# Arlo0o/StereoScene

Measured on AMD Instinct MI355X. Metric: voxels/sec fwd+bwd, 256x256x32 grid D=192, higher is better.
Workload: dtype f32; 1 GPU; kitti_d192: stereo pair features 2x[B,640,48,160] -> 256x256x32 occupancy, D=192, fwd+bwd incl. 4 losses; batch_per_gpu=1, global_batch=1, parallelism=dp1, train_mode=True

## Files before the change

### include/ssbev.h

```cpp
#ifndef SSBEV_H
#define SSBEV_H

#include <stddef.h>
#include <stdint.h>

#ifdef __cplusplus
extern "C" {
#endif

#define SSBEV_OK 0
#define SSBEV_EINVAL (-1)
#define SSBEV_EWORKSPACE (-2)
#define SSBEV_ELAUNCH (-3)

typedef void* ssbev_stream_t;

int ssbev_version(void);
const char* ssbev_build_arch(void);
void ssbev_env_refresh(void);

typedef struct {
  int B;
  int P;
  int C;
// ... 36 lines not shown
                         const int32_t* vox, float* grad_depth, float* grad_feat,
                         const ssbev_pool_dims* d, const ssbev_lift_dims* l, ssbev_stream_t stream);

typedef struct { int B, C, G, D, H, W; float down; int align_corners; } ssbev_gwc_dims;
int ssbev_gwc_warp_fwd(const float* left, const float* right, const float* calib, float* vol,
                       const ssbev_gwc_dims* d, ssbev_stream_t stream);
int ssbev_gwc_warp_bwd(const float* grad_vol, const float* left, const float* right,
                       const float* calib, float* grad_left, float* grad_right,
                       const ssbev_gwc_dims* d, ssbev_stream_t stream);
size_t ssbev_gwc_warp_bwd_workspace(const ssbev_gwc_dims* d);
int ssbev_gwc_warp_bwd_fused(const float* grad_vol, const float* left, const float* right,
                             const float* calib, float* grad_left, float* grad_right,
                             const ssbev_gwc_dims* d, void* workspace, size_t ws_bytes, ssbev_stream_t stream);

typedef struct {
  int B, Cin, Cout;
  int Di, Hi, Wi;
  int Do, Ho, Wo;
  int kd, kh, kw;
  int sd, sh, sw;
  int pd, ph, pw;
  int dd, dh, dw;
  int transposed;
  int relu;
  int accumulate;
  int tile_hint;
  int precision;
} ssbev_conv_dims;

size_t ssbev_conv_packed_weight_elems(const ssbev_conv_dims* d);
int ssbev_conv_kernel_class(const ssbev_conv_dims* d, int mode);
int ssbev_conv_chunk_groups(const ssbev_conv_dims* d, int mode);

size_t ssbev_conv_thin_workspace(const ssbev_conv_dims* d, int mode);
size_t ssbev_conv_thin_packed_elems(const ssbev_conv_dims* d, int mode);
int ssbev_conv_thin_pack(const float* w_src, float* w_packed, const ssbev_conv_dims* d, int mode, ssbev_stream_t stream);
int ssbev_conv_thin_run(const float* x, const float* w_packed, const float* bias, float* y, const ssbev_conv_dims* d,
                        int mode, void* workspace, size_t ws_bytes, ssbev_stream_t stream);
int ssbev_conv_pack_weight(const float* w_src, float* w_packed, const ssbev_conv_dims* d, int mode,
                           ssbev_stream_t stream);
int ssbev_conv_fwd(const float* x, const float* w_packed, const float* bias, float* y,
                   const ssbev_conv_dims* d, ssbev_stream_t stream);
int ssbev_conv_fwd_bf16(const uint16_t* x, const float* w_packed, const float* bias, void* y,
                        const ssbev_conv_dims* d, ssbev_stream_t stream);
int ssbev_conv_bwd_data_bf16(const uint16_t* gy, const float* w_packed_t, void* gx,
                             const ssbev_conv_dims* d, ssbev_stream_t stream);
int ssbev_conv_bwd_weight_bf16(const uint16_t* x, const uint16_t* gy, float* gw, const ssbev_conv_dims* d,
                               void* ws, size_t ws_bytes, ssbev_stream_t stream);
int ssbev_conv_bwd_data(const float* gy, const float* w_packed_t, float* gx,
                        const ssbev_conv_dims* d, ssbev_stream_t stream);
size_t ssbev_conv_bwd_weight_workspace(const ssbev_conv_dims* d);
int ssbev_conv_bwd_weight(const float* x, const float* gy, float* gw, const ssbev_conv_dims* d,
                          void* ws, size_t ws_bytes, ssbev_stream_t stream);

typedef struct { int M, N, K, batch; int out_fp32; } ssbev_gemm16_dims;
size_t ssbev_gemm16_packed_elems(const ssbev_gemm16_dims* d);
int ssbev_gemm16_pack(const float* B, uint16_t* packed, const ssbev_gemm16_dims* d, ssbev_stream_t stream);
int ssbev_gemm16_nn(const uint16_t* A, const uint16_t* packed, void* C, const ssbev_gemm16_dims* d, ssbev_stream_t stream);
size_t ssbev_gemm16_tn_workspace(const ssbev_gemm16_dims* d);
int ssbev_gemm16_tn(const uint16_t* A, const uint16_t* B, float* C, const ssbev_gemm16_dims* d, float* workspace,
                    size_t workspace_elems, ssbev_stream_t stream);

typedef struct { int B, C, G; int64_t S; float eps; int relu; int stats_given; int pre_act; int64_t ld_y, ld_gy; int io_dtype; } ssbev_norm_dims;
size_t ssbev_groupnorm_workspace(const ssbev_norm_dims* d);
int ssbev_groupnorm_fwd(const float* x, const float* gamma, const float* beta, const float* residual,
                        float* y, float* mean, float* rstd, const ssbev_norm_dims* d, void* ws,
                        size_t ws_bytes, ssbev_stream_t stream);
int ssbev_groupnorm_bwd(const float* gy, const float* x, const float* y, const float* gamma,
                        const float* mean, const float* rstd, float* gx, float* gresidual,
                        float* ggamma, float* gbeta, const ssbev_norm_dims* d, void* ws,
                        size_t ws_bytes, ssbev_stream_t stream);
size_t ssbev_groupnorm_mask_words(const ssbev_norm_dims* d);
int ssbev_groupnorm_fwd_mask(const float* x, const float* gamma, const float* beta, const float* residual, float* y,
                             float* mean, float* rstd, uint64_t* relu_mask, const ssbev_norm_dims* d, void* ws,
                             size_t ws_bytes, ssbev_stream_t stream);
int ssbev_groupnorm_bwd_mask(const float* gy, const float* x, const uint64_t* relu_mask, const float* gamma,
                             const float* mean, const float* rstd, float* gx, float* gresidual, float* ggamma, float* gbeta,
                             const ssbev_norm_dims* d, void* ws, size_t ws_bytes, ssbev_stream_t stream);

typedef struct { float* running_mean; float* running_var; float momentum; int64_t n; } ssbev_norm_ext;
int ssbev_groupnorm_fwd_ext(const float* x, const float* gamma, const float* beta, const float* residual, float* y,
                            float* mean, float* rstd, uint64_t* relu_mask, const ssbev_norm_dims* d,
                            const ssbev_norm_ext* ext, void* ws, size_t ws_bytes, ssbev_stream_t stream);
int ssbev_groupnorm_bwd_ext(const float* gy, const float* x, const float* y, const uint64_t* relu_mask, const float* gamma,
                            const float* mean, const float* rstd, float* gx, float* gresidual, float* ggamma, float* gbeta,
                            const ssbev_norm_dims* d, const ssbev_norm_ext* ext, void* ws, size_t ws_bytes,
                            ssbev_stream_t stream);

typedef struct { int B, C, Ga, Gb; int64_t S; float eps_a, eps_b; int relu; int a_batch, b_batch; int io_dtype;  } ssbev_norm2_dims;
size_t ssbev_groupnorm2_workspace(const ssbev_norm2_dims* d);
int ssbev_groupnorm2_fwd(const float* xa, const float* gamma_a, const float* beta_a, float* mean_a, float* rstd_a,
                         const float* xb, const float* gamma_b, const float* beta_b, float* mean_b, float* rstd_b, float* y,
                         uint64_t* relu_mask, const ssbev_norm2_dims* d, void* ws, size_t ws_bytes, ssbev_stream_t stream);
int ssbev_groupnorm2_bwd(const float* gy, const uint64_t* relu_mask, const float* xa, const float* gamma_a, const float* mean_a,
                         const float* rstd_a, const float* xb, const float* gamma_b, const float* mean_b, const float* rstd_b,
                         float* gxa, float* gxb, float* ggamma_a, float* gbeta_a, float* ggamma_b, float* gbeta_b,
                         const ssbev_norm2_dims* d, void* ws, size_t ws_bytes, ssbev_stream_t stream);

typedef struct { float* running_mean_a; float* running_var_a; float momentum_a;
                 float* running_mean_b; float* running_var_b; float momentum_b; } ssbev_norm2_ext;
int ssbev_groupnorm2_fwd_ext(const float* xa, const float* gamma_a, const float* beta_a, float* mean_a, float* rstd_a,
                             const float* xb, const float* gamma_b, const float* beta_b, float* mean_b, float* rstd_b, float* y,
                             uint64_t* relu_mask, const ssbev_norm2_dims* d, const ssbev_norm2_ext* ext, void* ws, size_t ws_bytes,
                             ssbev_stream_t stream);
int ssbev_groupnorm2_bwd_ext(const float* gy, const uint64_t* relu_mask, const float* xa, const float* gamma_a, const float* mean_a,
                             const float* rstd_a, const float* xb, const float* gamma_b, const float* mean_b, const float* rstd_b,
// ... 214 lines not shown
```

### stereoscene_amd/capi.py

```python
import ctypes as C
import os

import torch

_HERE = os.path.dirname(os.path.abspath(__file__))
LIB_PATH = os.path.join(_HERE, "_lib", "libssbev_hip.so")

OK, EINVAL, EWORKSPACE, ELAUNCH = 0, -1, -2, -3
_ERR = {EINVAL: "SSBEV_EINVAL (bad dims / null pointer / unsupported configuration)",
        EWORKSPACE: "SSBEV_EWORKSPACE (workspace too small)",
        ELAUNCH: "SSBEV_ELAUNCH (HIP launch failure)"}


class SsbevError(RuntimeError):
    pass


class PoolDims(C.Structure):
    _fields_ = [("B", C.c_int), ("P", C.c_int), ("C", C.c_int), ("nx", C.c_int), ("ny", C.c_int), ("nz", C.c_int),
                ("origin", C.c_float * 3), ("dx", C.c_float * 3)]


class LiftDims(C.Structure):
    _fields_ = [("N", C.c_int), ("D", C.c_int), ("HW", C.c_int)]
# ... 78 lines not shown
    _fields_ = [("kernel", C.c_int), ("bm", C.c_int), ("bn", C.c_int), ("bk", C.c_int), ("nchunk", C.c_int), ("per_chunk", C.c_int),
                ("grid", C.c_int64), ("workspace", C.c_size_t)]


class JitterParams(C.Structure):
    _fields_ = [("flags", C.c_int), ("mode", C.c_int), ("delta", C.c_float), ("alpha", C.c_float), ("saturation", C.c_float),
                ("hue", C.c_float), ("perm", C.c_int * 3)]


JITTER_BRIGHTNESS, JITTER_CONTRAST, JITTER_SATURATION, JITTER_HUE, JITTER_SWAP = 1, 2, 4, 8, 16


class AdamWCfg(C.Structure):
    _fields_ = [("lr", C.c_float), ("beta1", C.c_float), ("beta2", C.c_float), ("eps", C.c_float),
                ("weight_decay", C.c_float), ("max_grad_norm", C.c_float), ("step", C.c_int)]


_P = C.c_void_p
SIGNATURES = {
    "ssbev_version": (C.c_int, []),
    "ssbev_build_arch": (C.c_char_p, []),
    "ssbev_env_refresh": (None, []),
    "ssbev_voxel_index": (C.c_int, [_P, _P, _P, C.POINTER(PoolDims), _P]),
    "ssbev_coords_to_vox": (C.c_int, [_P, C.c_int, _P, C.POINTER(PoolDims), _P]),
    "ssbev_pool_prepare_workspace": (C.c_size_t, [C.c_int, C.POINTER(PoolDims)]),
    "ssbev_pool_prepare": (C.c_int, [_P, C.c_int, _P, _P, C.POINTER(PoolDims), _P, C.c_size_t, _P]),
    "ssbev_pool_long_list_elems": (C.c_size_t, [C.c_int]),
    "ssbev_pool_prepare2": (C.c_int, [_P, C.c_int, _P, _P, _P, C.POINTER(PoolDims), _P, C.c_size_t, _P]),
    "ssbev_bev_pool_fwd": (C.c_int, [_P, _P, _P, _P, C.POINTER(PoolDims), _P]),
    "ssbev_bev_pool_bwd": (C.c_int, [_P, _P, C.c_int, _P, C.POINTER(PoolDims), _P]),
    "ssbev_lift_splat_fwd": (C.c_int, [_P, _P, _P, _P, _P, C.POINTER(PoolDims), C.POINTER(LiftDims), _P]),
    "ssbev_lift_splat_fwd2": (C.c_int, [_P, _P, _P, _P, _P, _P, C.POINTER(PoolDims), C.POINTER(LiftDims), _P]),
    "ssbev_lift_splat_bwd": (C.c_int, [_P, _P, _P, _P, _P, _P, C.POINTER(PoolDims), C.POINTER(LiftDims), _P]),
    "ssbev_gwc_warp_fwd": (C.c_int, [_P, _P, _P, _P, C.POINTER(GwcDims), _P]),
    "ssbev_gwc_warp_bwd": (C.c_int, [_P, _P, _P, _P, _P, _P, C.POINTER(GwcDims), _P]),
    "ssbev_gwc_warp_bwd_workspace": (C.c_size_t, [C.POINTER(GwcDims)]),
    "ssbev_gwc_warp_bwd_fused": (C.c_int, [_P, _P, _P, _P, _P, _P, C.POINTER(GwcDims), _P, C.c_size_t, _P]),
    "ssbev_conv_packed_weight_elems": (C.c_size_t, [C.POINTER(ConvDims)]),
    "ssbev_conv_kernel_class": (C.c_int, [C.POINTER(ConvDims), C.c_int]),
    "ssbev_conv_chunk_groups": (C.c_int, [C.POINTER(ConvDims), C.c_int]),
    "ssbev_frustum_geometry": (C.c_int, [_P] * 9 + [C.POINTER(GeomDims), _P]),
    "ssbev_conv_pack_weight": (C.c_int, [_P, _P, C.POINTER(ConvDims), C.c_int, _P]),
    "ssbev_conv_thin_workspace": (C.c_size_t, [C.POINTER(ConvDims), C.c_int]),
    "ssbev_conv_thin_packed_elems": (C.c_size_t, [C.POINTER(ConvDims), C.c_int]),
    "ssbev_conv_thin_pack": (C.c_int, [_P, _P, C.POINTER(ConvDims), C.c_int, _P]),
    "ssbev_conv_thin_run": (C.c_int, [_P, _P, _P, _P, C.POINTER(ConvDims), C.c_int, _P, C.c_size_t, _P]),
    "ssbev_conv_fwd": (C.c_int, [_P, _P, _P, _P, C.POINTER(ConvDims), _P]),
    "ssbev_conv_bwd_data": (C.c_int, [_P, _P, _P, C.POINTER(ConvDims), _P]),
    "ssbev_conv_fwd_bf16": (C.c_int, [_P, _P, _P, _P, C.POINTER(ConvDims), _P]),
    "ssbev_conv_bwd_data_bf16": (C.c_int, [_P, _P, _P, C.POINTER(ConvDims), _P]),
    "ssbev_conv_bwd_weight_bf16": (C.c_int, [_P, _P, _P, C.POINTER(ConvDims), _P, C.c_size_t, _P]),
    "ssbev_conv_bwd_weight_workspace": (C.c_size_t, [C.POINTER(ConvDims)]),
    "ssbev_conv_bwd_weight": (C.c_int, [_P, _P, _P, C.POINTER(ConvDims), _P, C.c_size_t, _P]),
    "ssbev_gemm16_packed_elems": (C.c_size_t, [C.POINTER(Gemm16Dims)]),
    "ssbev_gemm16_pack": (C.c_int, [_P, _P, C.POINTER(Gemm16Dims), _P]),
    "ssbev_gemm16_nn": (C.c_int, [_P, _P, _P, C.POINTER(Gemm16Dims), _P]),
    "ssbev_gemm16_tn_workspace": (C.c_size_t, [C.POINTER(Gemm16Dims)]),
    "ssbev_gemm16_tn": (C.c_int, [_P, _P, _P, C.POINTER(Gemm16Dims), _P, C.c_size_t, _P]),
    "ssbev_groupnorm_workspace": (C.c_size_t, [C.POINTER(NormDims)]),
    "ssbev_groupnorm_fwd": (C.c_int, [_P] * 7 + [C.POINTER(NormDims), _P, C.c_size_t, _P]),
    "ssbev_groupnorm_bwd": (C.c_int, [_P] * 10 + [C.POINTER(NormDims), _P, C.c_size_t, _P]),
    "ssbev_groupnorm_mask_words": (C.c_size_t, [C.POINTER(NormDims)]),
    "ssbev_groupnorm_fwd_mask": (C.c_int, [_P] * 8 + [C.POINTER(NormDims), _P, C.c_size_t, _P]),
    "ssbev_groupnorm_bwd_mask": (C.c_int, [_P] * 10 + [C.POINTER(NormDims), _P, C.c_size_t, _P]),
    "ssbev_groupnorm_fwd_ext": (C.c_int, [_P] * 8 + [C.POINTER(NormDims), C.POINTER(NormExt), _P, C.c_size_t, _P]),
    "ssbev_groupnorm_bwd_ext": (C.c_int, [_P] * 11 + [C.POINTER(NormDims), C.POINTER(NormExt), _P, C.c_size_t, _P]),
    "ssbev_groupnorm2_fwd_ext": (C.c_int, [_P] * 12 + [C.POINTER(Norm2Dims), C.POINTER(Norm2Ext), _P, C.c_size_t, _P]),
    "ssbev_groupnorm2_bwd_ext": (C.c_int, [_P] * 16 + [C.POINTER(Norm2Dims), C.POINTER(Norm2Ext), _P, C.c_size_t, _P]),
    "ssbev_groupnorm2_workspace": (C.c_size_t, [C.POINTER(Norm2Dims)]),
    "ssbev_groupnorm2_fwd": (C.c_int, [_P] * 12 + [C.POINTER(Norm2Dims), _P, C.c_size_t, _P]),
    "ssbev_groupnorm2_bwd": (C.c_int, [_P] * 16 + [C.POINTER(Norm2Dims), _P, C.c_size_t, _P]),
    "ssbev_groupnorm_plan_query": (C.c_int, [C.POINTER(NormDims), C.POINTER(Norm2Dims), C.c_int, C.POINTER(GroupnormPlan)]),
    "ssbev_trilinear2x_fwd": (C.c_int, [_P, _P, C.POINTER(UpsampleDims), _P]),
    "ssbev_trilinear2x_bwd": (C.c_int, [_P, _P, C.POINTER(UpsampleDims), _P]),
    "ssbev_dcn_im2col": (C.c_int, [_P, _P, _P, C.POINTER(DcnDims), _P]),
    "ssbev_dcn_col2im_workspace": (C.c_size_t, [C.POINTER(DcnDims)]),
    "ssbev_dcn_col2im": (C.c_int, [_P, _P, _P, _P, _P, C.POINTER(DcnDims), _P, C.c_size_t, _P]),
    "ssbev_bn_update_running": (C.c_int, [_P, _P, _P, _P, C.c_int, C.c_float, C.c_float, C.c_int64, _P]),
    "ssbev_resize_pil_u8": (C.c_int, [_P, C.c_int, C.c_int, C.c_int, _P, _P, C.c_int, _P, _P, C.c_int, _P, _P, C.c_int, C.c_int, _P]),
    "ssbev_crop_normalize_u8": (C.c_int, [_P, C.c_int, C.c_int, _P, C.c_int, C.c_int, C.c_int, C.c_int, C.c_int, _P, _P, C.c_int, _P]),
    "ssbev_crop_rotate_normalize_u8": (C.c_int, [_P, C.c_int, C.c_int, _P, C.c_int, C.c_int, C.c_int, C.c_int, C.c_int, _P, _P, _P,
                                                C.c_int, _P]),
    "ssbev_crop_rotate_jitter_normalize_u8": (C.c_int, [_P, C.c_int, C.c_int, _P, C.c_int, C.c_int, C.c_int, C.c_int, C.c_int, _P,
                                                       C.POINTER(JitterParams), _P, _P, C.c_int, _P]),
    "ssbev_depth_bce_workspace": (C.c_size_t, [C.c_int, C.c_int, C.c_int]),
    "ssbev_depth_bce_fwd": (C.c_int, [_P, _P, _P] + [C.c_int] * 5 + [C.c_float] * 3 + [_P, C.c_size_t, _P]),
    "ssbev_depth_bce_bwd": (C.c_int, [_P, _P, _P, _P] + [C.c_int] * 5 + [C.c_float] * 3 + [_P, _P]),
    "ssbev_lidar_depth_workspace": (C.c_size_t, [C.c_int, C.c_int]),
    "ssbev_lidar_depth_map": (C.c_int, [_P, C.c_int, _P, _P, _P, _P, _P, _P, C.c_int, C.c_int, _P, C.c_size_t, _P]),
    "ssbev_dwconv2d_fwd": (C.c_int, [_P, _P, _P, C.POINTER(DwDims), _P]),
    "ssbev_dwconv2d_bwd_data": (C.c_int, [_P, _P, _P, C.POINTER(DwDims), _P]),
    "ssbev_dwconv2d_bwd_weight_workspace": (C.c_size_t, [C.POINTER(DwDims)]),
    "ssbev_dwconv2d_bwd_weight": (C.c_int, [_P, _P, _P, C.POINTER(DwDims), _P, C.c_size_t, _P]),
    "ssbev_swish_fwd": (C.c_int, [_P, _P, C.c_int64, _P]),
    "ssbev_swish_bwd": (C.c_int, [_P, _P, _P, C.c_int64, _P]),
    "ssbev_chan_sum_workspace": (C.c_size_t, [C.c_int, C.c_int64, C.c_int]),
    "ssbev_chan_sum": (C.c_int, [_P, _P, _P, C.c_int, C.c_int64, C.c_int, C.c_float, _P, C.c_size_t, _P]),
    "ssbev_chan_scale": (C.c_int, [_P, _P, _P, C.c_int, C.c_int64, C.c_int, C.c_float, _P]),
    "ssbev_wino_input_transform": (C.c_int, [_P, _P, C.POINTER(WinoDims), _P]),
    "ssbev_wino_output_transform": (C.c_int, [_P, _P, C.POINTER(WinoDims), _P]),
    "ssbev_wino_output_adjoint": (C.c_int, [_P, _P, C.POINTER(WinoDims), _P]),
    "ssbev_wino_weight_transform": (C.c_int, [_P, _P, C.c_int, C.c_int, C.c_int, C.c_int, _P]),
    "ssbev_wino_weight_grad": (C.c_int, [_P, _P, C.c_int, C.c_int, C.c_int, _P]),
    "ssbev_wino_dgemm_packed_elems": (C.c_size_t, [C.c_int, C.c_int]),
    "ssbev_wino_dgemm_pack": (C.c_int, [_P, _P, C.c_int, C.c_int, C.c_int, _P]),
    "ssbev_wino_dgemm": (C.c_int, [_P, _P, _P, C.POINTER(WinoDims), C.c_int, _P]),
# ... 117 lines not shown
```

### stereoscene_amd/csrc/capi.hip

```cpp
#include "common.h"

#include <cstdlib>
#include <mutex>
#include <string>
#include <unordered_map>

namespace {
struct EnvTable {
  std::mutex mu;
  std::unordered_map<std::string, std::pair<bool, std::string>> seen;
};
EnvTable& env_table() {
  static EnvTable* t = new EnvTable();
  return *t;
}
}

const char* ssbev_env(const char* name) {
  EnvTable& t = env_table();
  std::lock_guard<std::mutex> lock(t.mu);
  auto it = t.seen.find(name);
  if (it == t.seen.end()) {
    const char* v = std::getenv(name);
    it = t.seen.emplace(name, std::make_pair(v != nullptr, std::string(v ? v : ""))).first;
  }
  return it->second.first ? it->second.second.c_str() : nullptr;
}

extern "C" {
int ssbev_version(void) { return 107;  }
const char* ssbev_build_arch(void) { return "gfx950"; }

void ssbev_env_refresh(void) {
  EnvTable& t = env_table();
  std::lock_guard<std::mutex> lock(t.mu);
  t.seen.clear();
}
}
```

### stereoscene_amd/functional.py

```python
import ctypes as C

import os

import numpy as np
import torch

from . import capi, streams



class KernelTimer:

    def __init__(self, families=None):
        self.records = []
        self.counts = {}
        self.families = families

    def span(self, family, flops, nbytes=0.0, tag=None, executed=None):
        c = self.counts.setdefault(family, dict(launches=0, flops=0.0, bytes=0.0, executed=0.0))
        c["launches"] += 1
        c["flops"] += flops
        c["bytes"] += nbytes
        c["executed"] += flops if executed is None else executed
        if self.families is not None and family.split(":")[0] not in self.families:
# ... 417 lines not shown

def _slot_target(slot, like):
    if slot is None or slot.buf is None:
        return None
    b = slot.buf
    ok = b.is_contiguous() and b.dtype == like.dtype and b.numel() == like.numel() and b.shape[-1] == like.shape[-1] and \
        b.shape[0] == like.shape[0]
    return b.view(tuple(like.shape)) if ok else None




def _triple(v, n):
    if isinstance(v, int):
        return (v,) * n
    v = tuple(int(a) for a in v)
    return v if len(v) == n else (v[0],) * n


TILE_HINT = int(os.environ.get("SSBEV_TILE_HINT", "0"))


def _conv_dims(xshape_cl, wshape, stride, padding, dilation, transposed, output_padding, relu=0, accumulate=0):
    B, Di, Hi, Wi, Cin = xshape_cl
    kd, kh, kw = wshape[2:]
    if transposed:
        Cout = wshape[1]
        outs = [(i - 1) * s - 2 * p + dl * (k - 1) + op + 1
                for i, s, p, dl, k, op in zip((Di, Hi, Wi), stride, padding, dilation, (kd, kh, kw), output_padding)]
    else:
        Cout = wshape[0]
        outs = [(i + 2 * p - dl * (k - 1) - 1) // s + 1
                for i, s, p, dl, k in zip((Di, Hi, Wi), stride, padding, dilation, (kd, kh, kw))]
    d = capi.ConvDims(B, Cin, Cout, Di, Hi, Wi, outs[0], outs[1], outs[2], kd, kh, kw, *stride, *padding, *dilation,
                      int(transposed), int(relu), int(accumulate), int(TILE_HINT), 1 if PRECISION == "bf16_operands" else 0)
    return d


def _packed(weight5, d, mode):
    lib = capi.load()
    wp = torch.empty(lib.ssbev_conv_packed_weight_elems(C.byref(d)), dtype=torch.float32, device=weight5.device)
    capi.check(lib.ssbev_conv_pack_weight(capi.ptr(weight5.contiguous()), capi.ptr(wp), C.byref(d), mode,
                                          capi.stream()), "ssbev_conv_pack_weight")
    return wp


def _thin_out_run(lib, src, weight5, bias, out, d, mode):
    wp = torch.empty(lib.ssbev_conv_thin_packed_elems(C.byref(d), mode), dtype=torch.float32, device=src.device)
    capi.check(lib.ssbev_conv_thin_pack(capi.ptr(weight5.contiguous()), capi.ptr(wp), C.byref(d), mode, capi.stream()),
               "ssbev_conv_thin_pack")
    ws = _ws(lib.ssbev_conv_thin_workspace(C.byref(d), mode), src.device)
    capi.check(lib.ssbev_conv_thin_run(capi.ptr(src), capi.ptr(wp), capi.ptr(bias), capi.ptr(out), C.byref(d), mode,
                                       capi.ptr(ws), ws.numel(), capi.stream()), "ssbev_conv_thin_run")


class _ConvNd(torch.autograd.Function):

    @staticmethod
    def forward(ctx, x, weight, bias, stride, padding, dilation, transposed, output_padding, slot=None, relu=False):
        lib = capi.load()
        ctx.slot = slot
        if ctx.needs_input_grad[1]:
            streams.note_use(weight)
        xcl = to_cl(_f32(x, "conv"))
        kpad = (-xcl.shape[-1]) % 4
        w5 = weight
        thin_in = False
        if kpad and not transposed:
            d0 = _conv_dims(tuple(xcl.shape), tuple(weight.shape), stride, padding, dilation, transposed, output_padding)
            thin_in = lib.ssbev_conv_kernel_class(C.byref(d0), 0) == 4
        if kpad and not thin_in:
            xcl = torch.nn.functional.pad(xcl, (0, kpad))
            w5 = torch.nn.functional.pad(weight, (0, 0, 0, 0, 0, 0) + ((0, 0, 0, kpad) if transposed else (0, kpad)))
        d = _conv_dims(tuple(xcl.shape), tuple(w5.shape), stride, padding, dilation, transposed, output_padding, relu=int(relu))
        y = torch.empty(d.B, d.Do, d.Ho, d.Wo, d.Cout, dtype=torch.float32, device=x.device)
        b = bias.detach().contiguous() if bias is not None else None
        fam = _conv_family(lib, d, 0)
        with _span(fam, conv_flops(d), conv_bytes(d), _conv_tag(d, "fwd"), conv_flops(d) / _EXEC_DIV[fam]):
            if lib.ssbev_conv_kernel_class(C.byref(d), 0) == 5:
                _thin_out_run(lib, xcl, w5.detach(), b, y, d, 0)
            else:
                wp = _packed(w5.detach(), d, 0)
                capi.check(lib.ssbev_conv_fwd(capi.ptr(xcl), capi.ptr(wp), capi.ptr(b), capi.ptr(y), C.byref(d),
                                              capi.stream()), "ssbev_conv_fwd")
        ctx.relu = bool(relu)
        ctx.save_for_backward(xcl, weight, *((y,) if relu else ()))
        ctx.cfg = (stride, padding, dilation, transposed, output_padding, 0 if thin_in else kpad, bias is not None)
        ctx.thin_in = thin_in
        ctx.bias_leaf = bias is not None and bias.is_leaf and bias.grad is None
        return from_cl(y)

    @staticmethod
    def backward(ctx, gy):
        lib = capi.load()
        xcl, weight = ctx.saved_tensors[:2]
        stride, padding, dilation, transposed, output_padding, kpad, has_bias = ctx.cfg
        args = (stride, padding, dilation, transposed, output_padding)
        if ctx.relu:
            ycl = ctx.saved_tensors[2]
            gy = from_cl(torch.ops.aten.threshold_backward(to_cl(gy).contiguous(), ycl, 0.0))
        gcl0 = to_cl(gy)
        Cout_g = gcl0.shape[-1]
        cpad = (-Cout_g) % 4
        tpad = (-xcl.shape[-1]) % 4 if ctx.thin_in else 0
        want_gx, want_gw = ctx.needs_input_grad[0], ctx.needs_input_grad[1]
        thin_d = thin_w = False
        d0 = None
        if not transposed and not kpad and (cpad or tpad):
            d0 = _conv_dims(tuple(xcl.shape), tuple(weight.shape), *args)
            thin_d = bool(cpad) and lib.ssbev_conv_kernel_class(C.byref(d0), 1) == 4
            thin_w = lib.ssbev_conv_kernel_class(C.byref(d0), 2) == 6
        w5 = weight.detach()
        if kpad:
            w5 = torch.nn.functional.pad(w5, (0, 0, 0, 0, 0, 0) + ((0, 0, 0, kpad) if transposed else (0, kpad)))
        gcl = gcl0
        if cpad and ((want_gx and not thin_d) or (want_gw and not thin_w)):
            gcl = torch.nn.functional.pad(gcl0, (0, cpad))
            w5 = torch.nn.functional.pad(w5, (0, 0, 0, 0, 0, 0) + ((0, cpad) if transposed else (0, 0, 0, cpad)))
        elif cpad:
            w5 = None
        d = _conv_dims(tuple(xcl.shape), tuple(w5.shape), *args) if w5 is not None else d0
        gx = gw = gb = None

        def weight_gradient():
            pointwise = (not transposed and tuple(weight.shape[2:]) == (1, 1, 1) and stride == (1, 1, 1) and padding == (0, 0, 0)
                         and not kpad and not cpad and not tpad and weight.shape[0] <= 128 and weight.shape[1] <= 128
                         and gcl0.numel() // Cout_g >= 32768)
            if pointwise and OWN_GEMM and PRECISION == "fp32":
                with _span("conv_wgrad", conv_flops(d), conv_bytes(d), _conv_tag(d, "wgrad")):
                    gw = gemm_tn(gcl0.reshape(-1, Cout_g), xcl.reshape(-1, xcl.shape[-1])).view_as(weight)
            else:
                if thin_w:
                    xw, gw_src, dw, wshape = xcl, gcl0, d0, tuple(weight.shape)
                else:
                    xw, gw_src, dw, wshape = xcl, gcl, d, tuple(w5.shape)
                    if tpad:
                        xw = torch.nn.functional.pad(xcl, (0, tpad))
                        wshape = (wshape[0], wshape[1] + tpad) + wshape[2:]
                        dw = _conv_dims(tuple(xw.shape), wshape, *args)
                gwp = torch.empty(wshape, dtype=torch.float32, device=gy.device)
                ws = _ws(lib.ssbev_conv_bwd_weight_workspace(C.byref(dw)), gy.device)
                with _span("conv_wgrad", conv_flops(dw), conv_bytes(dw), _conv_tag(dw, "wgrad")):
                    capi.check(lib.ssbev_conv_bwd_weight(capi.ptr(xw), capi.ptr(gw_src), capi.ptr(gwp), C.byref(dw),
                                                         capi.ptr(ws), ws.numel(), capi.stream()),
                               "ssbev_conv_bwd_weight")
                gw = gwp if tuple(wshape) == tuple(weight.shape) else gwp[: weight.shape[0], : weight.shape[1]].contiguous()
            return gw

        gw_side = want_gw and streams.wgrad_on_side(weight)
        want_gb = has_bias and ctx.needs_input_grad[2]
        gb_side = gw_side and want_gb and ctx.bias_leaf
        if gw_side:
            with streams.on_side(gy.device, xcl, gcl0, gcl) as side:
                gw = weight_gradient()
                if gb_side:
                    gb = gcl0.reshape(-1, Cout_g).sum(0)
                side.publish(gw, gb)
        if want_gx:
            dd, gdl, wd = (d0, gcl0, weight.detach()) if thin_d else (d, gcl, w5)
            slot = ctx.slot if (not kpad and not thin_d and lib.ssbev_conv_kernel_class(C.byref(dd), 1) not in (4, 5)) else None
            into = _slot_target(slot, xcl)
            if into is not None:
                dd.accumulate = 1
            gxcl = into if into is not None else torch.empty_like(xcl)
            fam = _conv_family(lib, dd, 1)
            with _span(fam, conv_flops(dd), conv_bytes(dd), _conv_tag(dd, "dgrad"), conv_flops(dd) / _EXEC_DIV[fam]):
                if lib.ssbev_conv_kernel_class(C.byref(dd), 1) == 5:
                    _thin_out_run(lib, gdl, wd, None, gxcl, dd, 1)
                else:
                    wpt = _packed(wd, dd, 1)
                    capi.check(lib.ssbev_conv_bwd_data(capi.ptr(gdl), capi.ptr(wpt), capi.ptr(gxcl), C.byref(dd),
                                                       capi.stream()), "ssbev_conv_bwd_data")
            dd.accumulate = 0
            if slot is not None:
                slot.buf = gxcl
            if kpad:
                gxcl = gxcl[..., : xcl.shape[-1] - kpad]
            gx = from_cl(gxcl)
        if want_gw and not gw_side:
            gw = weight_gradient()
        if want_gb and not gb_side:
            gb = gcl0.reshape(-1, Cout_g).sum(0)
        return gx, gw, gb, None, None, None, None, None, None, None


class _ConvNd16(torch.autograd.Function):

    @staticmethod
    def forward(ctx, x, weight, bias, stride, padding, dilation, transposed, output_padding, slot=None, relu=False, out_fp32=False):
        lib = capi.load()
        ctx.slot = slot
        if ctx.needs_input_grad[1]:
            streams.note_use(weight)
        xcl = to_cl(x if x.dtype == torch.bfloat16 else x.to(torch.bfloat16))
        d = _conv_dims(tuple(xcl.shape), tuple(weight.shape), stride, padding, dilation, transposed, output_padding, relu=int(relu))
        d.precision = 3 if out_fp32 else 2
        y = torch.empty(d.B, d.Do, d.Ho, d.Wo, d.Cout, dtype=torch.float32 if out_fp32 else torch.bfloat16, device=x.device)
        b = bias.detach().float().contiguous() if bias is not None else None
        fam = {17: "conv_tap16", 19: "conv_wide16"}.get(lib.ssbev_conv_kernel_class(C.byref(d), 0), "conv_gather16") if KERNEL_TIMER is not None else "conv_gather16"
        with _span(fam, conv_flops(d), conv_bytes(d) / 2.0, _conv_tag(d, "fwd")):
            wp = _packed(weight.detach(), d, 0)
            capi.check(lib.ssbev_conv_fwd_bf16(capi.ptr(xcl), capi.ptr(wp), capi.ptr(b), capi.ptr(y), C.byref(d), capi.stream()),
                       "ssbev_conv_fwd_bf16")
        ctx.relu = bool(relu)
        ctx.save_for_backward(xcl, weight, *((y,) if relu else ()))
        ctx.cfg = (stride, padding, dilation, transposed, output_padding, bias is not None)
        ctx.bias_leaf = bias is not None and bias.is_leaf and bias.grad is None
        return from_cl(y)

    @staticmethod
    def backward(ctx, gy):
        lib = capi.load()
        xcl, weight = ctx.saved_tensors[:2]
        stride, padding, dilation, transposed, output_padding, has_bias = ctx.cfg
        gcl = to_cl(gy)
        if ctx.relu:
            gcl = torch.ops.aten.threshold_backward(gcl.contiguous(), ctx.saved_tensors[2], 0.0)
        if gcl.dtype != torch.bfloat16:
            gcl = gcl.to(torch.bfloat16)
        Cout_g = gcl.shape[-1]
        d = _conv_dims(tuple(xcl.shape), tuple(weight.shape), stride, padding, dilation, transposed, output_padding)
# ... 172 lines not shown
    lib = capi.load()
    ws = _ws(lib.ssbev_gemm_nn_workspace(C.byref(g)), a.device)
    with _span("gemm_own", fl, 4.0 * (a.numel() + b.numel() + out.numel()), tag or f"nn {batch}x{M}x{K}x{N}"):
        capi.check(lib.ssbev_gemm_nn(_rawptr(a), _rawptr(b), _rawptr(bias.contiguous() if bias is not None else None),
                                     capi.ptr(out), C.byref(g), capi.ptr(ws), ws.numel(), capi.stream()), "ssbev_gemm_nn")
    return out


def gemm_nt(a, w, bias=None, relu=False, tag=None):
    if not _gemm_supported(a, w) or a.shape[-1] % 4 or w.shape[-2] % 4:
        y = torch.matmul(a, w.transpose(-1, -2))
        y = y if bias is None else y + bias
        return torch.relu(y) if relu else y
    a, lda, sa = _rows(a)
    w, ldb, sb = _rows(w)
    batch = a.shape[0] if a.dim() == 3 else 1
    M, K, N = a.shape[-2], a.shape[-1], w.shape[-2]
    out = torch.empty(*a.shape[:-1], N, dtype=torch.float32, device=a.device)
    g = _gdims(M, N, K, batch, lda, ldb, N, sa, sb if w.dim() == 3 else 0, M * N, relu)
    fl = 2.0 * batch * M * N * K
    lib = capi.load()
    ws = _ws(lib.ssbev_gemm_nt_workspace(C.byref(g)), a.device)
    with _span("gemm_own", fl, 4.0 * (a.numel() + w.numel() + out.numel()), tag or f"nt {batch}x{M}x{K}x{N}"):
        capi.check(lib.ssbev_gemm_nt(_rawptr(a), _rawptr(w), _rawptr(bias.contiguous() if bias is not None else None),
                                     capi.ptr(out), C.byref(g), capi.ptr(ws), ws.numel(), capi.stream()), "ssbev_gemm_nt")
    return out


def gemm_tn(a, b, tag=None, ep_mul=None, ep_rowsub=None):
    if not _gemm_supported(a, b) or a.shape[-1] % 4 or b.shape[-1] % 4:
        c = torch.matmul(a.transpose(-1, -2), b)
        return c if ep_mul is None else ep_mul * (c - ep_rowsub.unsqueeze(-1))
    a, lda, sa = _rows(a)
    b, ldb, sb = _rows(b)
    batch = a.shape[0] if a.dim() == 3 else 1
    R, K, N = a.shape[-2], a.shape[-1], b.shape[-1]
    out = torch.empty(*a.shape[:-2], K, N, dtype=torch.float32, device=a.device)
    g = _gdims(R, N, K, batch, lda, ldb, N, sa, sb, K * N)
    if ep_mul is not None:
        ep_mul, ep_rowsub = ep_mul.contiguous(), ep_rowsub.contiguous().float()
        if tuple(ep_mul.shape) != tuple(out.shape) or ep_rowsub.numel() != batch * K:
            raise capi.SsbevError("gemm_tn: epilogue operand shapes")
        g.ep_mul, g.ep_rowsub = ep_mul.data_ptr(), ep_rowsub.data_ptr()
    lib = capi.load()
    ws = _ws(lib.ssbev_gemm_tn_workspace(C.byref(g)), a.device)
    fl = 2.0 * batch * R * N * K
    with _span("gemm_own", fl, 4.0 * (a.numel() + b.numel() + out.numel() * (2 if ep_mul is not None else 1)),
               tag or f"tn {batch}x{R}x{K}x{N}"):
        capi.check(lib.ssbev_gemm_tn(_rawptr(a), _rawptr(b), capi.ptr(out), C.byref(g), capi.ptr(ws), ws.numel(), capi.stream()),
                   "ssbev_gemm_tn")
    return out


class _LinearCL(torch.autograd.Function):

    @staticmethod
    def forward(ctx, x2, w2, bias):
        ctx.save_for_backward(x2, w2)
        ctx.has_bias = bias is not None
        return gemm_nt(x2, w2, bias, tag=f"linear fwd {w2.shape[1]}->{w2.shape[0]} rows={x2.shape[0]}")

    @staticmethod
    def backward(ctx, gy):
        x2, w2 = ctx.saved_tensors
        gy = gy.contiguous()
        gx = gw = gb = None
        if ctx.needs_input_grad[0]:
            gx = gemm_nn(gy, w2, tag=f"linear dgrad {w2.shape[1]}->{w2.shape[0]} rows={x2.shape[0]}")
        if ctx.needs_input_grad[1]:
            gw = gemm_tn(gy, x2, tag=f"linear wgrad {w2.shape[1]}->{w2.shape[0]} rows={x2.shape[0]}")
        if ctx.has_bias and ctx.needs_input_grad[2]:
            gb = gy.sum(0)
        return gx, gw, gb


_D2S_TABLES = {}


def _d2s_table(B, D, H, W, k, Co, device):
    key = (B, D, H, W, k, Co, str(device))
    t = _D2S_TABLES.get(key)
    if t is None:
        t = torch.empty(B * D * H * W, dtype=torch.int64, device=device)
        capi.check(capi.load().ssbev_gemm_d2s_rowoff(capi.ptr(t), B * D * H * W, D, H, W, k[0], k[1], k[2], Co, capi.stream()),
                   "ssbev_gemm_d2s_rowoff")
        _D2S_TABLES[key] = t
    return t


class _DeconvKS(torch.autograd.Function):

    @staticmethod
    def forward(ctx, xcl, weight, bias, k):
        B, D, H, W, Ci = xcl.shape
        Co = weight.shape[1]
        kd, kh, kw = k
        taps = kd * kh * kw
        wk = weight.detach().permute(0, 2, 3, 4, 1).reshape(Ci, taps * Co).contiguous()
        table = _d2s_table(B, D, H, W, k, Co, xcl.device)
        y = torch.empty(B, D * kd, H * kh, W * kw, Co, dtype=torch.float32, device=xcl.device)
        x2 = xcl.reshape(-1, Ci)
        R = x2.shape[0]
        g = _gdims(R, taps * Co, Ci, 1, Ci, taps * Co, 0, 0, 0, 0, 0, ((D, H, W, kd, kh, kw, Co), table))
        fl = 2.0 * R * Ci * taps * Co
        with _span("gemm_own", fl, 4.0 * (x2.numel() + wk.numel() + y.numel()), f"deconv k=s fwd {Ci}->{Co} k{kd}{kh}{kw}"):
            capi.check(capi.load().ssbev_gemm_nn(capi.ptr(x2), capi.ptr(wk), capi.ptr(bias.detach().contiguous() if bias is not None else None),
                                                 capi.ptr(y), C.byref(g), None, 0, capi.stream()), "ssbev_gemm_nn")
        ctx.save_for_backward(x2, wk)
        ctx.meta = (B, D, H, W, Ci, Co, k, bias is not None)
        return y

    @staticmethod
    def backward(ctx, gy):
        x2, wk = ctx.saved_tensors
        B, D, H, W, Ci, Co, k, has_bias = ctx.meta
        kd, kh, kw = k
        taps = kd * kh * kw
        gy = gy.contiguous()
        table = _d2s_table(B, D, H, W, k, Co, gy.device)
        d2s = ((D, H, W, kd, kh, kw, Co), table)
        R = x2.shape[0]
# ... 1346 lines not shown
```

Before: 30.60 million voxels/s.

## Add streaming MFMA pointwise kernel for 1x1x1 convs and large linears

```diff
diff --git a/include/ssbev.h b/include/ssbev.h
--- a/include/ssbev.h
+++ b/include/ssbev.h
@@ -112,6 +112,12 @@
 size_t ssbev_conv_bwd_weight_workspace(const ssbev_conv_dims* d);
 int ssbev_conv_bwd_weight(const float* x, const float* gy, float* gw, const ssbev_conv_dims* d,
                           void* ws, size_t ws_bytes, ssbev_stream_t stream);
+
+int ssbev_pointwise_applicable(int64_t M, int K, int N);
+size_t ssbev_pointwise_packed_elems(int K, int N);
+int ssbev_pointwise_pack(const float* w_src, float* w_packed, int K, int N, int mode, ssbev_stream_t stream);
+int ssbev_pointwise_run(const float* x, const float* w_packed, const float* bias, float* y, int64_t M, int K, int N,
+                        int relu, int accumulate, ssbev_stream_t stream);
 
 typedef struct { int M, N, K, batch; int out_fp32; } ssbev_gemm16_dims;
 size_t ssbev_gemm16_packed_elems(const ssbev_gemm16_dims* d);
diff --git a/stereoscene_amd/capi.py b/stereoscene_amd/capi.py
--- a/stereoscene_amd/capi.py
+++ b/stereoscene_amd/capi.py
@@ -154,6 +154,10 @@
     "ssbev_conv_bwd_weight_bf16": (C.c_int, [_P, _P, _P, C.POINTER(ConvDims), _P, C.c_size_t, _P]),
     "ssbev_conv_bwd_weight_workspace": (C.c_size_t, [C.POINTER(ConvDims)]),
     "ssbev_conv_bwd_weight": (C.c_int, [_P, _P, _P, C.POINTER(ConvDims), _P, C.c_size_t, _P]),
+    "ssbev_pointwise_applicable": (C.c_int, [C.c_int64, C.c_int, C.c_int]),
+    "ssbev_pointwise_packed_elems": (C.c_size_t, [C.c_int, C.c_int]),
+    "ssbev_pointwise_pack": (C.c_int, [_P, _P, C.c_int, C.c_int, C.c_int, _P]),
+    "ssbev_pointwise_run": (C.c_int, [_P, _P, _P, _P, C.c_int64, C.c_int, C.c_int, C.c_int, C.c_int, _P]),
     "ssbev_gemm16_packed_elems": (C.c_size_t, [C.POINTER(Gemm16Dims)]),
     "ssbev_gemm16_pack": (C.c_int, [_P, _P, C.POINTER(Gemm16Dims), _P]),
     "ssbev_gemm16_nn": (C.c_int, [_P, _P, _P, C.POINTER(Gemm16Dims), _P]),
diff --git a/stereoscene_amd/csrc/capi.hip b/stereoscene_amd/csrc/capi.hip
--- a/stereoscene_amd/csrc/capi.hip
+++ b/stereoscene_amd/csrc/capi.hip
@@ -28,7 +28,7 @@
 }
 
 extern "C" {
-int ssbev_version(void) { return 107;  }
+int ssbev_version(void) { return 108;  }
 const char* ssbev_build_arch(void) { return "gfx950"; }
 
 void ssbev_env_refresh(void) {
diff --git a/stereoscene_amd/csrc/pointwise_stream.hip b/stereoscene_amd/csrc/pointwise_stream.hip
--- /dev/null
+++ b/stereoscene_amd/csrc/pointwise_stream.hip
@@ -0,0 +1,265 @@
+#include "common.h"
+
+#include <cstdlib>
+
+namespace {
+
+typedef float f32x16 __attribute__((ext_vector_type(16)));
+
+__device__ __forceinline__ f32x16 mfma32(float a, float b, f32x16 c) {
+  return __builtin_amdgcn_mfma_f32_32x32x2f32(a, b, c, 0, 0, 0);
+}
+
+__device__ const float kPwZeros[4] = {0.f, 0.f, 0.f, 0.f};
+
+constexpr int kRing = 4;
+constexpr int kChunkF = 1024;
+constexpr int kMaxC = 192;
+constexpr int kMaxWeightRegs = 96;
+
+struct PwNGeom {
+  long M;
+  int K, N;
+  int nsl;
+  int relu, has_bias, accumulate;
+  long tpg;
+};
+
+struct PwNPlan {
+  int G, KC, SPW, nsl;
+};
+
+bool pwn_plan(long M, int K, int N, PwNPlan* p) {
+  if (M <= 0 || K < 4 || N < 4 || K > kMaxC || N > kMaxC || (K & 3) || (N & 3)) return false;
+  if (K <= 32 && N <= 32) return false;
+  const int nsl = (N + 31) / 32, KC = (K + 31) / 32;
+  const int G = nsl == 1 ? 1 : nsl == 2 ? 2 : 4;
+  const int SPW = (nsl + G - 1) / G;
+  if (KC * SPW * 16 > kMaxWeightRegs) return false;
+  if (p) *p = PwNPlan{G, KC, SPW, nsl};
+  return true;
+}
+
+__global__ void __launch_bounds__(256)
+pack_pwn_kernel(const float* __restrict__ w, float* __restrict__ wp, int K, int N, int KC, int total, int mode) {
+  const int i = blockIdx.x * 256 + threadIdx.x;
+  if (i >= total) return;
+  const int lane = i & 63, r = (i >> 6) & 15, blk = i >> 10;
+  const int kc = blk % KC, sl = blk / KC;
+  const int n = 32 * sl + (lane & 31), k = 32 * kc + 8 * (r >> 2) + 4 * (lane >> 5) + (r & 3);
+  float v = 0.0f;
+  if (n < N && k < K) v = mode == 0 ? w[(size_t)n * K + k] : w[(size_t)k * N + n];
+  wp[i] = v;
+}
+
+template <int N> __device__ __forceinline__ void wait_vm() {
+  static_assert(N >= 0 && N < 16, "vmcnt immediate");
+  __builtin_amdgcn_s_waitcnt(0x0F70 | N);
+  asm volatile("" ::: "memory");
+}
+
+template <int G, int KC, int SPW>
+__global__ void __launch_bounds__(64 * G)
+conv_pwN_kernel(const float* __restrict__ X, const float* __restrict__ wp, const float* __restrict__ bias,
+                float* __restrict__ Y, PwNGeom g) {
+  constexpr int IPW = 4 / G;
+  __shared__ __align__(16) float tl[(kRing + G) * kChunkF];
+  const int tid = threadIdx.x, lane = tid & 63;
+  const int wave = __builtin_amdgcn_readfirstlane(tid >> 6);
+  const int li = lane & 31, lk = lane >> 5;
+  float* outt = tl + (kRing + wave) * kChunkF;
+  float wr[SPW][KC][16];
+#pragma unroll
+  for (int j = 0; j < SPW; ++j) {
+    const int sl = min(wave + G * j, g.nsl - 1);
+#pragma unroll
+    for (int kc = 0; kc < KC; ++kc)
+#pragma unroll
+      for (int r = 0; r < 16; ++r) wr[j][kc][r] = wp[((sl * KC + kc) * 16 + r) * 64 + lane];
+  }
+  const int cq = lane & 7;
+  float bv[SPW][4];
+#pragma unroll
+  for (int j = 0; j < SPW; ++j)
+#pragma unroll
+    for (int i = 0; i < 4; ++i) {
+      const int n = 32 * (wave + G * j) + 4 * cq + i;
+      bv[j][i] = (g.has_bias && n < g.N) ? bias[n] : 0.0f;
+    }
+  const long ntiles = (g.M + 31) >> 5;
+  const long t0 = (long)blockIdx.x * g.tpg, t1 = min(ntiles, t0 + g.tpg);
+  const long S = (t1 - t0) * KC;
+  int su[IPW], sc[IPW];
+#pragma unroll
+  for (int i = 0; i < IPW; ++i) {
+    const int e = wave + G * i;
+    su[i] = e * 8 + (lane >> 3);
+    sc[i] = ((lane & 7) ^ ((su[i] >> 1) & 7)) << 2;
+  }
+  long st_t = t0;
+  int st_kc = 0, st_slot = 0;
+  auto stage = [&]() {
+    const long left = g.M - st_t * 32;
+    const float* base = X + st_t * 32 * (long)g.K + st_kc * 32;
+#pragma unroll
+    for (int i = 0; i < IPW; ++i) {
+      const float* src = (st_kc * 32 + sc[i] < g.K && su[i] < left) ? base + (long)su[i] * g.K + sc[i] : kPwZeros;
+      glds16(src, tl + st_slot * kChunkF + (wave + G * i) * 256);
+    }
+    if (++st_kc == KC) { st_kc = 0; ++st_t; }
+    if (++st_slot == kRing) st_slot = 0;
+  };
+  wait_vm0();
+  for (int j = 0; j < kRing - 1; ++j)
+    if (j < S) stage();
+  long s = 0;
+  int slot = 0;
+  for (long t = t0; t < t1; ++t) {
+    f32x16 acc[SPW];
+#pragma unroll
+    for (int j = 0; j < SPW; ++j)
+#pragma unroll
+      for (int r = 0; r < 16; ++r) acc[j][r] = 0.0f;
+#pragma unroll
+    for (int kc = 0; kc < KC; ++kc, ++s) {
+      if (s + kRing - 2 < S) wait_vm<(kRing - 2) * IPW>(); else wait_vm0();
+      if (G > 1) barrier_lds();
+      if (s + kRing - 1 < S) stage();
+      asm volatile("" ::: "memory");
+      const float* tp = tl + slot * kChunkF + li * 32;
+      const int sw = (li >> 1) & 7;
+#pragma unroll
+      for (int q = 0; q < 4; ++q) {
+        const float4 xv = *reinterpret_cast<const float4*>(tp + (((2 * q + lk) ^ sw) << 2));
+#pragma unroll
+        for (int j = 0; j < SPW; ++j) {
+          acc[j] = mfma32(wr[j][kc][4 * q + 0], xv.x, acc[j]);
+          acc[j] = mfma32(wr[j][kc][4 * q + 1], xv.y, acc[j]);
+          acc[j] = mfma32(wr[j][kc][4 * q + 2], xv.z, acc[j]);
+          acc[j] = mfma32(wr[j][kc][4 * q + 3], xv.w, acc[j]);
+        }
+      }
+      if (++slot == kRing) slot = 0;
+    }
+#pragma unroll
+    for (int j = 0; j < SPW; ++j) {
+      const int sl = wave + G * j;
+      if (sl >= g.nsl) continue;
+      const int nq = 32 * sl + 4 * cq;
+      const int sw = (li >> 1) & 7;
+#pragma unroll
+      for (int rq = 0; rq < 4; ++rq)
+        *reinterpret_cast<float4*>(outt + li * 32 + (((2 * rq + lk) ^ sw) << 2)) =
+            make_float4(acc[j][4 * rq], acc[j][4 * rq + 1], acc[j][4 * rq + 2], acc[j][4 * rq + 3]);
+      asm volatile("s_waitcnt lgkmcnt(0)" ::: "memory");
+      float4 ov[4];
+      if (g.accumulate) {
+#pragma unroll
+        for (int it = 0; it < 4; ++it) {
+          const long v = t * 32 + it * 8 + (lane >> 3);
+          ov[it] = (v < g.M && nq < g.N) ? *reinterpret_cast<const float4*>(Y + v * g.N + nq) : make_float4(0.f, 0.f, 0.f, 0.f);
+        }
+      }
+#pragma unroll
+      for (int it = 0; it < 4; ++it) {
+        const int u = it * 8 + (lane >> 3);
+        const long v = t * 32 + u;
+        const float4 a4 = *reinterpret_cast<const float4*>(outt + u * 32 + ((cq ^ ((u >> 1) & 7)) << 2));
+        float o[4] = {a4.x + bv[j][0], a4.y + bv[j][1], a4.z + bv[j][2], a4.w + bv[j][3]};
+        if (g.relu) {
+#pragma unroll
+          for (int i = 0; i < 4; ++i) o[i] = fmaxf(o[i], 0.0f);
+        }
+        if (g.accumulate) { o[0] += ov[it].x; o[1] += ov[it].y; o[2] += ov[it].z; o[3] += ov[it].w; }
+        if (v < g.M && nq < g.N) *reinterpret_cast<float4*>(Y + v * g.N + nq) = make_float4(o[0], o[1], o[2], o[3]);
+      }
+      asm volatile("s_waitcnt lgkmcnt(0)" ::: "memory");
+    }
+  }
+}
+
+template <int G, int KC, int SPW>
+void launch_pwn(const float* x, const float* wp, const float* bias, float* y, PwNGeom g, hipStream_t st) {
+  static const int resident = [] {
+    int n = 0;
+    if (hipOccupancyMaxActiveBlocksPerMultiprocessor(&n, conv_pwN_kernel<G, KC, SPW>, 64 * G, 0) != hipSuccess || n < 1) n = 2;
+    return n;
+  }();
+  const long ntiles = (g.M + 31) / 32, cap = 256L * resident;
+  long wgs;
+  if (ntiles <= cap * 4) wgs = (ntiles + 3) / 4;
+  else wgs = cap * ((ntiles + cap * 12 - 1) / (cap * 12));
+  g.tpg = (ntiles + wgs - 1) / wgs;
+  const unsigned nblocks = (unsigned)((ntiles + g.tpg - 1) / g.tpg);
+  hipLaunchKernelGGL((conv_pwN_kernel<G, KC, SPW>), dim3(nblocks), dim3(64 * G), 0, st, x, wp, bias, y, g);
+}
+
+template <int G, int SPW>
+bool launch_pwn_kc(int KC, const float* x, const float* wp, const float* bias, float* y, const PwNGeom& g, hipStream_t st) {
+  switch (KC) {
+    case 1: launch_pwn<G, 1, SPW>(x, wp, bias, y, g, st); return true;
+    case 2: launch_pwn<G, 2, SPW>(x, wp, bias, y, g, st); return true;
+    case 3: launch_pwn<G, 3, SPW>(x, wp, bias, y, g, st); return true;
+    default: break;
+  }
+  if constexpr (SPW == 1) {
+    switch (KC) {
+      case 4: launch_pwn<G, 4, 1>(x, wp, bias, y, g, st); return true;
+      case 5: launch_pwn<G, 5, 1>(x, wp, bias, y, g, st); return true;
+      case 6: launch_pwn<G, 6, 1>(x, wp, bias, y, g, st); return true;
+      default: break;
+    }
+  }
+  return false;
+}
+
+}
+
+extern "C" {
+
+int ssbev_pointwise_applicable(int64_t M, int K, int N) {
+  const char* env = ssbev_env("SSBEV_PW_STREAM");
+  if (env && atoi(env) == 0) return 0;
+  return pwn_plan((long)M, K, N, nullptr) ? 1 : 0;
+}
+
+size_t ssbev_pointwise_packed_elems(int K, int N) {
+  PwNPlan p;
+  if (!pwn_plan(1, K, N, &p)) return 0;
+  return (size_t)p.nsl * p.KC * 16 * 64;
+}
+
+int ssbev_pointwise_pack(const float* w_src, float* w_packed, int K, int N, int mode, ssbev_stream_t stream) {
+  PwNPlan p;
+  if (!w_src || !w_packed || (mode != 0 && mode != 1) || !pwn_plan(1, K, N, &p)) return SSBEV_EINVAL;
+  const int total = p.nsl * p.KC * 16 * 64;
+  hipLaunchKernelGGL(pack_pwn_kernel, dim3(cdiv((size_t)total, 256)), dim3(256), 0, as_stream(stream), w_src, w_packed, K, N,
+                     p.KC, total, mode);
+  return ssbev_launch_status();
+}
+
+int ssbev_pointwise_run(const float* x, const float* w_packed, const float* bias, float* y, int64_t M, int K, int N, int relu,
+                        int accumulate, ssbev_stream_t stream) {
+  PwNPlan p;
+  if (!x || !w_packed || !y || !pwn_plan((long)M, K, N, &p)) return SSBEV_EINVAL;
+  if (((uintptr_t)x | (uintptr_t)y | (uintptr_t)w_packed) & 15) return SSBEV_EINVAL;
+  PwNGeom g;
+  g.M = (long)M;
+  g.K = K;
+  g.N = N;
+  g.nsl = p.nsl;
+  g.relu = relu ? 1 : 0;
+  g.has_bias = bias ? 1 : 0;
+  g.accumulate = accumulate ? 1 : 0;
+  g.tpg = 0;
+  hipStream_t st = as_stream(stream);
+  bool ok = false;
+  if (p.G == 1) ok = launch_pwn_kc<1, 1>(p.KC, x, w_packed, bias, y, g, st);
+  else if (p.G == 2) ok = launch_pwn_kc<2, 1>(p.KC, x, w_packed, bias, y, g, st);
+  else if (p.SPW == 1) ok = launch_pwn_kc<4, 1>(p.KC, x, w_packed, bias, y, g, st);
+  else ok = launch_pwn_kc<4, 2>(p.KC, x, w_packed, bias, y, g, st);
+  if (!ok) return SSBEV_EINVAL;
+  return ssbev_launch_status();
+}
+
+}
diff --git a/stereoscene_amd/functional.py b/stereoscene_amd/functional.py
--- a/stereoscene_amd/functional.py
+++ b/stereoscene_amd/functional.py
@@ -493,6 +493,23 @@
     ws = _ws(lib.ssbev_conv_thin_workspace(C.byref(d), mode), src.device)
     capi.check(lib.ssbev_conv_thin_run(capi.ptr(src), capi.ptr(wp), capi.ptr(bias), capi.ptr(out), C.byref(d), mode,
                                        capi.ptr(ws), ws.numel(), capi.stream()), "ssbev_conv_thin_run")
+
+
+def _pw_stream_ok(lib, M, K, N):
+    return PRECISION == "fp32" and TILE_HINT == 0 and bool(lib.ssbev_pointwise_applicable(int(M), int(K), int(N)))
+
+
+def _pw_stream_run(lib, src, w2, bias, out, M, K, N, mode, relu=0, accumulate=0):
+    wp = torch.empty(lib.ssbev_pointwise_packed_elems(int(K), int(N)), dtype=torch.float32, device=src.device)
+    capi.check(lib.ssbev_pointwise_pack(capi.ptr(w2.contiguous()), capi.ptr(wp), int(K), int(N), mode, capi.stream()),
+               "ssbev_pointwise_pack")
+    capi.check(lib.ssbev_pointwise_run(capi.ptr(src), capi.ptr(wp), capi.ptr(bias), capi.ptr(out), int(M), int(K), int(N),
+                                       int(relu), int(accumulate), capi.stream()), "ssbev_pointwise_run")
+
+
+def _conv_is_pointwise(d):
+    return (not d.transposed and (d.kd, d.kh, d.kw) == (1, 1, 1) and (d.sd, d.sh, d.sw) == (1, 1, 1)
+            and (d.pd, d.ph, d.pw) == (0, 0, 0))
 
 
 class _ConvNd(torch.autograd.Function):
@@ -520,6 +537,9 @@
         with _span(fam, conv_flops(d), conv_bytes(d), _conv_tag(d, "fwd"), conv_flops(d) / _EXEC_DIV[fam]):
             if lib.ssbev_conv_kernel_class(C.byref(d), 0) == 5:
                 _thin_out_run(lib, xcl, w5.detach(), b, y, d, 0)
+            elif not kpad and x.is_cuda and _conv_is_pointwise(d) and _pw_stream_ok(lib, y.numel() // d.Cout, d.Cin, d.Cout):
+                _pw_stream_run(lib, xcl, w5.detach().reshape(d.Cout, d.Cin), b, y, y.numel() // d.Cout, d.Cin, d.Cout, 0,
+                               relu=int(relu))
             else:
                 wp = _packed(w5.detach(), d, 0)
                 capi.check(lib.ssbev_conv_fwd(capi.ptr(xcl), capi.ptr(wp), capi.ptr(b), capi.ptr(y), C.byref(d),
@@ -608,6 +628,10 @@
             with _span(fam, conv_flops(dd), conv_bytes(dd), _conv_tag(dd, "dgrad"), conv_flops(dd) / _EXEC_DIV[fam]):
                 if lib.ssbev_conv_kernel_class(C.byref(dd), 1) == 5:
                     _thin_out_run(lib, gdl, wd, None, gxcl, dd, 1)
+                elif (not kpad and not cpad and not thin_d and gy.is_cuda and _conv_is_pointwise(dd)
+                      and _pw_stream_ok(lib, gxcl.numel() // dd.Cin, dd.Cout, dd.Cin)):
+                    _pw_stream_run(lib, gdl.contiguous(), wd.reshape(dd.Cout, dd.Cin), None, gxcl, gxcl.numel() // dd.Cin, dd.Cout,
+                                   dd.Cin, 1, accumulate=dd.accumulate)
                 else:
                     wpt = _packed(wd, dd, 1)
                     capi.check(lib.ssbev_conv_bwd_data(capi.ptr(gdl), capi.ptr(wpt), capi.ptr(gxcl), C.byref(dd),
@@ -886,12 +910,34 @@
     return out
 
 
+PW_STREAM_MIN_ROWS = 262144
+
+
+def _linear_streams(x2, w2):
+    return (x2.is_cuda and x2.dtype == torch.float32 and w2.dtype == torch.float32 and x2.shape[0] >= PW_STREAM_MIN_ROWS
+            and x2.data_ptr() % 16 == 0 and _pw_stream_ok(capi.load(), x2.shape[0], w2.shape[1], w2.shape[0]))
+
+
+def _linear_stream(src, w2, bias, mode, tag):
+    lib = capi.load()
+    Cout, Cin = w2.shape
+    K, N = (Cin, Cout) if mode == 0 else (Cout, Cin)
+    src = src.contiguous()
+    M = src.shape[0]
+    out = torch.empty(M, N, dtype=torch.float32, device=src.device)
+    with _span("gemm_own", 2.0 * M * N * K, 4.0 * (src.numel() + w2.numel() + out.numel()), tag):
+        _pw_stream_run(lib, src, w2.detach(), bias.detach().contiguous() if bias is not None else None, out, M, K, N, mode)
+    return out
+
+
 class _LinearCL(torch.autograd.Function):
 
     @staticmethod
     def forward(ctx, x2, w2, bias):
         ctx.save_for_backward(x2, w2)
         ctx.has_bias = bias is not None
+        if _linear_streams(x2, w2):
+            return _linear_stream(x2, w2, bias, 0, f"linear fwd {w2.shape[1]}->{w2.shape[0]} rows={x2.shape[0]}")
         return gemm_nt(x2, w2, bias, tag=f"linear fwd {w2.shape[1]}->{w2.shape[0]} rows={x2.shape[0]}")
 
     @staticmethod
@@ -900,7 +946,10 @@
         gy = gy.contiguous()
         gx = gw = gb = None
         if ctx.needs_input_grad[0]:
-            gx = gemm_nn(gy, w2, tag=f"linear dgrad {w2.shape[1]}->{w2.shape[0]} rows={x2.shape[0]}")
+            if _linear_streams(x2, w2):
+                gx = _linear_stream(gy, w2, None, 1, f"linear dgrad {w2.shape[1]}->{w2.shape[0]} rows={x2.shape[0]}")
+            else:
+                gx = gemm_nn(gy, w2, tag=f"linear dgrad {w2.shape[1]}->{w2.shape[0]} rows={x2.shape[0]}")
         if ctx.needs_input_grad[1]:
             gw = gemm_tn(gy, x2, tag=f"linear wgrad {w2.shape[1]}->{w2.shape[0]} rows={x2.shape[0]}")
         if ctx.has_bias and ctx.needs_input_grad[2]:
```

Measured after the change: 30.81 million voxels/s (median of 6 runs). About the same (+0.7%).
